# iDC-NEU/NeutronStarLite

Measured on AMD Instinct MI355X. Metric: aggregated_edges_per_sec, higher is better.
Workload: dtype f32; 1 GPU; reddit: RMAT V=232965 E=114232965 feat=602 GCN-layer aggregation fwd+bwd (BASELINE config #2); model=gcn, V=232965, E=114232965, feat=602, relabel=none, parallelism=graph-partitioned dp1

## Files before the change

include/nts_hip.h:

```cpp
#ifndef NTS_HIP_H
#define NTS_HIP_H

#include <stdint.h>

#ifdef __cplusplus
extern "C" {
#endif

typedef uint32_t nts_vid;

typedef struct nts_stream nts_stream;

nts_stream *nts_stream_create(void);
nts_stream *nts_stream_wrap(void *hip_stream);
void nts_stream_destroy(nts_stream *s);
void nts_stream_sync(nts_stream *s);
void *nts_stream_handle(nts_stream *s);
void nts_stream_wait_stream(nts_stream *waiter, nts_stream *waitee);

enum nts_ktag {
  NTS_KTAG_FWD = 0,
  NTS_KTAG_BWD = 1,
  NTS_KTAG_DESER = 2,
  NTS_KTAG_AGGMSG = 3,
// ... 70 lines not shown
    int *grid, unsigned long long *scratch_bytes);

enum nts_gather_sched {
  NTS_SCHED_ITEM = 0,
  NTS_SCHED_PHASE = 1,
  NTS_SCHED_XCD = 2
};

void nts_gather_schedule(nts_stream *s, int schedule, int window_floats);

void nts_gather_schedule_last(nts_stream *s, int *schedule, int *window_floats);

void nts_gather_plan(nts_vid feature_size, unsigned alignment_bytes,
    nts_vid rows, nts_vid batch_size, nts_vid edges, int schedule_req,
    int window_req, int *schedule, int *window_floats, int *lane_group,
    int *vector_width, int *grid, int *blocked);

void nts_gather_plan_bf16(nts_vid feature_size, unsigned alignment_bytes,
    nts_vid rows, nts_vid batch_size, nts_vid edges, int schedule_req,
    int window_req, int *schedule, int *window_floats, int *lane_group,
    int *vector_width, int *grid, int *blocked);

void nts_gather_staging(nts_stream *s, int mode);

void nts_gather_staging_last(nts_stream *s, int *staged, int *pitch_floats);

void nts_gather_stage_plan(nts_vid feature_size, unsigned elem_bytes,
    unsigned in_alignment_bytes, unsigned out_alignment_bytes, nts_vid rows,
    nts_vid batch_size, nts_vid edges, int schedule_req, int window_req,
    int stage_req, int *staged, int *pitch_floats, int *schedule,
    int *window_floats, int *lane_group, int *vector_width, int *store_width,
    int *grid, int *blocked);

void nts_items_cache_clear(nts_stream *s);

void nts_deserialize_to_gpu(nts_stream *s, float *gpu_buffer, const float *msg,
    nts_vid count, nts_vid feature_size, nts_vid partition_start,
    nts_vid partition_end, int sync);

void nts_aggregate_comm_result(nts_stream *s, float *master, const float *msg,
    nts_vid count, nts_vid feature_size, nts_vid partition_start,
    nts_vid partition_end, int sync);

void nts_gather_rows(nts_stream *s, const float *dense, float *packed,
    const nts_vid *index, nts_vid count, nts_vid row_start, nts_vid feature_size);
void nts_scatter_rows(nts_stream *s, float *dense, const float *packed,
    const nts_vid *index, nts_vid count, nts_vid row_start, nts_vid feature_size);
void nts_scatter_add_rows(nts_stream *s, float *dense, const float *packed,
    const nts_vid *index, nts_vid count, nts_vid row_start, nts_vid feature_size);

void nts_scatter_src_mirror_to_msg(nts_stream *s, float *message,
    const float *src_mirror_feature, const nts_vid *row_indices,
    const nts_vid *column_offset, const nts_vid *mirror_index,
    nts_vid batch_size, nts_vid feature_size);
void nts_gather_msg_to_src_mirror(nts_stream *s, float *src_mirror_feature,
    const float *message, const nts_vid *row_indices,
    const nts_vid *column_offset, const nts_vid *mirror_index,
    nts_vid batch_size, nts_vid feature_size);
void nts_scatter_dst_to_msg(nts_stream *s, float *message,
    const float *dst_feature, const nts_vid *row_indices,
    const nts_vid *column_offset, nts_vid batch_size, nts_vid feature_size);
void nts_gather_msg_to_dst(nts_stream *s, float *dst_feature,
    const float *message, const nts_vid *row_indices,
    const nts_vid *column_offset, nts_vid batch_size, nts_vid feature_size);

void nts_edge_softmax_forward(nts_stream *s, float *msg_output,
// ... 84 lines not shown
```

neutronstarlite_amd/csrc/nts_hip.hip:

```cpp
#include <hip/hip_runtime.h>

#include <cstdio>
#include <cstdlib>
#include <cstring>
#include <map>
#include <utility>
#include <vector>

#include "../../include/nts_hip.h"

#define NTS_CHECK(cmd)                                                        \
  do {                                                                        \
    hipError_t e_ = (cmd);                                                    \
    if (e_ != hipSuccess) {                                                   \
      fprintf(stderr, "nts_hip: %s failed: %s (%s:%d)\n", #cmd,               \
              hipGetErrorString(e_), __FILE__, __LINE__);                     \
      abort();          \
    }                                                                         \
  } while (0)

namespace {
constexpr int NTS_BLOCK = 256;

uint32_t env_u32(const char *name, uint32_t dflt) {
// ... 21 lines not shown
  uint4 *items = nullptr;
  uint32_t *counter = nullptr;
  uint64_t cap = 0;
  const uint32_t *key_off = nullptr;
  uint32_t key_batch = 0, key_edges = 0;
  bool valid = false;
};
}

struct nts_stream {
  hipStream_t stream = nullptr;
  bool owned = false;
  bool timing = false;
  struct Rec { hipEvent_t a, b; int tag; };
  std::vector<Rec> pending;
  std::vector<std::pair<hipEvent_t, hipEvent_t>> freeev;
  double acc_ns[NTS_KTAG_COUNT] = {};
  long long acc_n[NTS_KTAG_COUNT] = {};
  ItemsBuf items_scratch[2];
  int items_rr = 0;
  bool items_reuse = false;
  int sched_req = 0, window_req = 0;
  int sched_last = 0, window_last = 0;
  float *sums_ws = nullptr;
  uint64_t sums_cap = 0;
  unsigned long long *keys_ws = nullptr;
  uint64_t keys_cap = 0;
  float *stage_ws = nullptr;
  uint64_t stage_cap = 0;
  int stage_req = 0;
  bool staged_last = false;
  uint32_t stage_ld_last = 0;
  bool heads_general = false;
};

namespace {
struct Tic {
  nts_stream *s;
  int tag;
  hipEvent_t a = nullptr, b = nullptr;
  Tic(nts_stream *s_, int tag_) : s(s_), tag(tag_) {
    if (!s->timing) return;
    if (!s->freeev.empty()) {
      a = s->freeev.back().first;
      b = s->freeev.back().second;
      s->freeev.pop_back();
    } else {
      NTS_CHECK(hipEventCreate(&a));
      NTS_CHECK(hipEventCreate(&b));
    }
    NTS_CHECK(hipEventRecord(a, s->stream));
  }
  ~Tic() {
    if (!s->timing || !a) return;
    NTS_CHECK(hipEventRecord(b, s->stream));
    s->pending.push_back({a, b, tag});
  }
};

void drain_timing(nts_stream *s) {
  if (s->pending.empty()) return;
  NTS_CHECK(hipStreamSynchronize(s->stream));
  for (auto &r : s->pending) {
    float ms = 0.f;
    NTS_CHECK(hipEventElapsedTime(&ms, r.a, r.b));
    s->acc_ns[r.tag] += (double)ms * 1e6;
// ... 319 lines not shown
          for (int j = 0; j < nv; ++j) acc[j] = fmaf(w, to_f32(p[j]), acc[j]);
        }
      }
      if (nv > 0)
        store_acc<ELEM, OV>(out + (uint64_t)im.v * f + col, acc, nv,
                            im.shared);
    }
  }
}

template <int SV>
__global__ __launch_bounds__(NTS_BLOCK) void k_repitch(
    const float *__restrict__ src, float *__restrict__ dst, uint32_t rows,
    uint32_t f, uint32_t ld) {
  const WaveId w = wave_id();
  for (uint32_t r = w.wave; r < rows; r += w.n_waves) {
    const float *s = src + (uint64_t)r * f;
    float *d = dst + (uint64_t)r * ld;
    for (uint32_t c = w.lane * 4; c < f; c += 64 * 4) {
      fvec<4> v;
      if (c + 4 <= f) {
#pragma unroll
        for (int k = 0; k < 4 / SV; ++k) {
          const fvec<SV> x = *reinterpret_cast<const fvec<SV> *>(s + c + k * SV);
#pragma unroll
          for (int j = 0; j < SV; ++j) v[k * SV + j] = x[j];
        }
      } else {
#pragma unroll
        for (int j = 0; j < 4; ++j) v[j] = (c + j < f) ? s[c + j] : 0.f;
      }
      *reinterpret_cast<fvec<4> *>(d + c) = v;
    }
  }
}

template <int ELEM, int NE>
__device__ __forceinline__ void heads_edges_vec(float (&acc)[ELEM],
                                                const GatherSrc<float> &g,
                                                uint32_t e, uint32_t col,
                                                uint32_t K, uint32_t head) {
  const float *p[NE];
  float wv[NE];
#pragma unroll
  for (int k = 0; k < NE; ++k) {
    p[k] = g.in + (uint64_t)(g.nbr[e + k] - g.nbr_start) * g.ld + col;
    wv[k] = g.ew[(uint64_t)(e + k) * K + head];
  }
  fma_vec<ELEM, NE>(acc, p, wv);
}
template <int NSTR, int NE>
__device__ __forceinline__ void heads_edges_strided(
    float (&acc)[NSTR], const GatherSrc<float> &g, uint32_t e, uint32_t col,
    uint32_t G, uint32_t K, const uint32_t (&hd)[NSTR]) {
  const float *p[NE];
  const float *wrow[NE];
#pragma unroll
  for (int k = 0; k < NE; ++k) {
    p[k] = g.in + (uint64_t)(g.nbr[e + k] - g.nbr_start) * g.ld + col;
    wrow[k] = g.ew + (uint64_t)(e + k) * K;
  }
#pragma unroll
  for (int k = 0; k < NE; ++k)
#pragma unroll
    for (int j = 0; j < NSTR; ++j)
      if (col + j * G < g.f)
// ... 958 lines not shown
  NTS_CHECK(hipMemsetAsync(ib.counter, 0, sizeof(uint32_t), s->stream));
  {
    Tic t(s, NTS_KTAG_ITEMS);
    hipLaunchKernelGGL(k_build_items, dim3(grid_for(batch)), dim3(NTS_BLOCK), 0,
                       s->stream, offset, batch, NTS_SPLIT, ib.items,
                       ib.counter);
  }
  dbg_sync(s, "k_build_items");
  ib.key_off = offset;
  ib.key_batch = batch;
  ib.key_edges = edges;
  ib.valid = s->items_reuse;
  return ib;
}

uint32_t items_grid(uint32_t batch, uint32_t edges) {
  return grid_for(((uint64_t)batch + edges / NTS_SPLIT) * 64);
}

constexpr uint64_t NTS_BLOCK_MIN_BYTES = 256ull << 20;
constexpr uint32_t NTS_BLOCK_MIN_REUSE = 32;
constexpr int NTS_AUTO_SCHED = NTS_SCHED_PHASE;
constexpr uint32_t NTS_AUTO_WINDOW = 0;
constexpr int NTS_AUTO_SCHED_BF16 = NTS_SCHED_XCD;
constexpr uint32_t NTS_AUTO_WINDOW_BF16 = 302;
constexpr int NTS_AUTO_SCHED_STAGED = NTS_SCHED_PHASE;
constexpr uint32_t NTS_AUTO_WINDOW_STAGED = 128;

struct GatherEnv {
  bool forced = false;
  int sched = 0, window = 0;
  int stage = 0;
  uint32_t stage_pitch = 0;
  uint32_t split, max_blocks, gather_blocks;
};
const GatherEnv &gather_env() {
  static const GatherEnv env = [] {
    GatherEnv v;
    const char *e = getenv("NTS_GATHER_SCHED");
    if (e && *e && atoi(e) >= 0) {
      v.forced = true;
      v.sched = atoi(e);
      const char *w = getenv("NTS_GATHER_WINDOW");
      if (w && *w) v.window = atoi(w);
    }
    const char *st = getenv("NTS_GATHER_STAGE");
    if (st && *st) v.stage = atoi(st) > 0 ? 1 : atoi(st) < 0 ? -1 : 0;
    v.stage_pitch = env_u32("NTS_GATHER_STAGE_PITCH", 0);
    v.split = NTS_SPLIT;
    v.max_blocks = NTS_MAX_BLOCKS;
    v.gather_blocks = nts_gather_blocks();
    return v;
  }();
  return env;
}

struct GatherGeom { int elem, nstr; uint32_t G; };
GatherGeom gather_geometry(uint32_t f, uintptr_t alignment,
                           uint32_t elem_bytes, uint32_t also_divides = 0) {
  GatherGeom g;
  g.elem = 1;
  for (uint32_t bytes = 16; bytes > elem_bytes; bytes /= 2) {
    const uint32_t n = bytes / elem_bytes;
    if (f % n == 0 && alignment % bytes == 0 &&
        (!also_divides || also_divides % n == 0)) {
      g.elem = (int)n;
      break;
    }
  }
  g.nstr = (g.elem == 1) ? 4 : 1;
  const uint32_t unit = g.elem * g.nstr;
  const uint32_t need = (f + unit - 1) / unit;
  g.G = 64;
  while (g.G / 2 >= need && g.G > 16) g.G /= 2;
  return g;
}

struct GatherLaunch {
  int elem;
  uint32_t G, grid;
  bool blocked;
// ... 90 lines not shown
};
StagePlan plan_stage(uint32_t f, uint32_t elem_bytes, uintptr_t in_alignment,
                     uintptr_t out_alignment, uint32_t rows, uint32_t batch,
                     uint32_t edges, int sched_req, int window_req,
                     int stage_req, const GatherEnv &env) {
  const int req = stage_req ? stage_req : env.stage;
  const uint32_t unit =
      env.stage_pitch ? (env.stage_pitch + 3u) / 4u * 4u : NTS_STAGE_PITCH_UNIT;
  const uint64_t ld = ((uint64_t)f + unit - 1) / unit * unit;
  bool staged = elem_bytes == sizeof(float) && rows && req >= 0 &&
                ld <= 0xffffffffu &&
                (uint64_t)rows * ld * sizeof(float) <= NTS_STAGE_MAX_BYTES;
  if (staged && req == 0) {
    const GatherGeom native =
        gather_geometry(f, in_alignment | out_alignment, elem_bytes);
    const uint32_t slabf = native.G * native.elem * native.nstr;
    staged = ld != f && f > slabf &&
             (uint64_t)rows * f * elem_bytes > NTS_BLOCK_MIN_BYTES &&
             edges / NTS_STAGE_MIN_REUSE >= rows;
  }
  if (!staged) {
    const GatherLaunch L =
        plan_gather(f, in_alignment | out_alignment, elem_bytes, rows, batch,
                    edges, sched_req, window_req, env);
    return StagePlan{false, f, common_ov(L.elem, (int)elem_bytes), L};
  }
  GatherGeom geo{4, 1, 64};
  while (geo.G / 2 >= (f + 3) / 4 && geo.G > 16) geo.G /= 2;
  return StagePlan{true, (uint32_t)ld, stage_store_width(f, out_alignment),
                   plan_gather(geo, f, elem_bytes, rows, batch, edges,
                               sched_req, window_req, env, true)};
}

float *get_stage(nts_stream *s, uint64_t n) {
  if (s->stage_cap < n) {
    NTS_CHECK(hipStreamSynchronize(s->stream));
    if (s->stage_ws) NTS_CHECK(hipFree(s->stage_ws));
    s->stage_ws = nullptr;
    s->stage_cap = 0;
    NTS_CHECK(hipMalloc(&s->stage_ws, n * sizeof(float)));
    s->stage_cap = n;
  }
  return s->stage_ws;
}

template <typename T>
void launch_gather(nts_stream *s, const T *in, float *out, const float *ew,
                   const uint32_t *nbr, const uint32_t *offset,
                   uint32_t nbr_start, uint32_t batch, uint32_t edges,
                   uint32_t f, int with_weight, int tag, uint32_t rows) {
  if (!batch || !edges || !f) return;
  ItemsBuf &ib = get_items(s, offset, batch, edges);
  const StagePlan P = plan_stage(f, sizeof(T), (uintptr_t)in, (uintptr_t)out,
                                 rows, batch, edges, s->sched_req,
                                 s->window_req, s->stage_req, gather_env());
  const GatherLaunch &L = P.L;
  using Kernel = decltype(&k_gather_spmm<T, 1, false, false>);
#define NTS_K(E)                                                              \
  {{k_gather_spmm<T, E, false, false>, k_gather_spmm<T, E, false, true>},     \
   {k_gather_spmm<T, E, true, false>, k_gather_spmm<T, E, true, true>}}
  constexpr int WIDEST = 16 / (int)sizeof(T);
  static const Kernel kernels[4][2][2] = {NTS_K(1), NTS_K(2), NTS_K(4),
                                          NTS_K(WIDEST)};
#undef NTS_K
  s->sched_last = (int)L.pl.sched;
  s->window_last = (int)L.pl.wf;
  s->staged_last = P.staged;
  s->stage_ld_last = P.staged ? P.ld : 0;
  if constexpr (sizeof(T) == sizeof(float)) {
    if (P.staged) {
#define NTS_K(OV)                                                             \
  {{k_gather_spmm<float, 4, false, false, OV>,                                \
    k_gather_spmm<float, 4, false, true, OV>},                                \
   {k_gather_spmm<float, 4, true, false, OV>,                                 \
    k_gather_spmm<float, 4, true, true, OV>}}
      static const Kernel staged_kernels[3][2][2] = {NTS_K(1), NTS_K(2),
                                                     NTS_K(4)};
#undef NTS_K
      float *stage = get_stage(s, (uint64_t)rows * P.ld);
      const int sv = stage_store_width(f, (uintptr_t)in);
      Tic t(s, tag);
      hipLaunchKernelGGL(sv == 4   ? k_repitch<4>
                         : sv == 2 ? k_repitch<2>
                                   : k_repitch<1>,
                         dim3(grid_for((uint64_t)rows * 64)), dim3(NTS_BLOCK),
                         0, s->stream, in, stage, rows, f, P.ld);
      hipLaunchKernelGGL(staged_kernels[__builtin_ctz((unsigned)P.ov)]
                                       [with_weight != 0][L.blocked],
                         dim3(L.grid), dim3(NTS_BLOCK), 0, s->stream, ib.items,
                         ib.counter, nbr, ew, (const float *)stage, out,
                         nbr_start, f, P.ld, L.G, L.pl);
      dbg_sync(s, "k_gather_spmm (staged)");
      return;
    }
  }
  Tic t(s, tag);
  hipLaunchKernelGGL(kernels[__builtin_ctz((unsigned)L.elem)]
                            [with_weight != 0][L.blocked],
                     dim3(L.grid), dim3(NTS_BLOCK), 0, s->stream, ib.items,
                     ib.counter, nbr, ew, in, out, nbr_start, f, f, L.G, L.pl);
  dbg_sync(s, "k_gather_spmm");
}

void check_heads(const char *entry, uint32_t f, uint32_t heads) {
  if (heads == 0 || heads > f || f % heads != 0) {
    fprintf(stderr, "%s: heads %u does not divide feature_size %u\n", entry,
            heads, f);
    abort();
  }
}

GatherLaunch plan_gather_heads(uint32_t f, uint32_t heads, uintptr_t alignment,
                               uint32_t batch, uint32_t edges,
                               const GatherEnv &env) {
  const GatherGeom geo =
      gather_geometry(f, alignment, sizeof(float), f / heads);
  const uint32_t slabf = geo.G * geo.elem * geo.nstr;
  const uint32_t n_slabs = (f + slabf - 1) / slabf;
  const uint64_t bound_items = (uint64_t)batch + edges / env.split + 1;
  return GatherLaunch{
      geo.elem, geo.G,
      grid_for(bound_items * n_slabs * geo.G, env.max_blocks), false,
      GatherPlan{NTS_SCHED_ITEM, slabf, n_slabs, 1u}};
}

void launch_gather_heads(nts_stream *s, const char *entry, const float *in,
                         float *out, const float *ew, const uint32_t *nbr,
                         const uint32_t *offset, uint32_t nbr_start,
                         uint32_t batch, uint32_t edges, uint32_t f,
                         uint32_t heads, int tag, uint32_t rows) {
  check_heads(entry, f, heads);
  if (heads == 1) {
    launch_gather(s, in, out, ew, nbr, offset, nbr_start, batch, edges, f, 1,
                  tag, rows);
    return;
  }
  if (!batch || !edges) return;
  ItemsBuf &ib = get_items(s, offset, batch, edges);
  const GatherLaunch L = plan_gather_heads(
      f, heads, (uintptr_t)in | (uintptr_t)out, batch, edges, gather_env());
  s->sched_last = (int)L.pl.sched;
  s->window_last = (int)L.pl.wf;
  Tic t(s, tag);
  hipLaunchKernelGGL(L.elem == 4   ? k_gather_spmm_heads<4>
                     : L.elem == 2 ? k_gather_spmm_heads<2>
                                   : k_gather_spmm_heads<1>,
                     dim3(L.grid), dim3(NTS_BLOCK), 0, s->stream, ib.items,
                     ib.counter, nbr, ew, in, out, nbr_start, f, L.G,
                     L.pl.n_windows, heads, f / heads);
  dbg_sync(s, "k_gather_spmm_heads");
}

void check_reduce_op(const char *entry, int op) {
  if (op != NTS_REDUCE_MAX && op != NTS_REDUCE_MIN) {
    fprintf(stderr, "%s: op %d is neither NTS_REDUCE_MAX nor NTS_REDUCE_MIN\n",
            entry, op);
    abort();
  }
}

struct ReduceLaunch {
  GatherLaunch L;
  uint64_t key_elems;
};
ReduceLaunch plan_reduce(uint32_t f, uintptr_t alignment, uint32_t batch,
                         uint32_t edges, const GatherEnv &env) {
  ReduceLaunch r{};
  if (!batch || !edges || !f) return r;
  r.L = plan_gather(f, alignment, sizeof(float), batch, batch, edges,
                    NTS_SCHED_ITEM, -1, env);
  r.key_elems = edges > env.split ? (uint64_t)batch * f : 0;
  return r;
}

unsigned long long *get_keys(nts_stream *s, uint64_t n) {
  if (s->keys_cap < n) {
    NTS_CHECK(hipStreamSynchronize(s->stream));
    if (s->keys_ws) NTS_CHECK(hipFree(s->keys_ws));
    NTS_CHECK(hipMalloc(&s->keys_ws, n * sizeof(unsigned long long)));
    s->keys_cap = n;
  }
  return s->keys_ws;
}

void launch_reduce(nts_stream *s, int op, const float *in, float *out,
                   uint32_t *arg, const uint32_t *nbr, const uint32_t *offset,
                   uint32_t nbr_start, uint32_t batch, uint32_t edges,
                   uint32_t f) {
  check_reduce_op("nts_reduce_by_dst_from_src", op);
  if (!batch || !f) return;
  const ReduceLaunch R = plan_reduce(
      f, (uintptr_t)in | (uintptr_t)out | (uintptr_t)arg, batch, edges,
      gather_env());
  ItemsBuf *ib = edges ? &get_items(s, offset, batch, edges) : nullptr;
  unsigned long long *keys = R.key_elems ? get_keys(s, R.key_elems) : nullptr;
  const uint32_t row_grid = grid_for((uint64_t)batch * 64);
  s->sched_last = NTS_SCHED_ITEM;
  s->window_last = (int)R.L.pl.wf;
  Tic t(s, NTS_KTAG_FWD);
  hipLaunchKernelGGL((k_reduce_rows<false, false>), dim3(row_grid),
                     dim3(NTS_BLOCK), 0, s->stream, offset, batch, NTS_SPLIT,
                     out, arg, keys, f);
  if (ib) {
    using Kernel = decltype(&k_gather_reduce<1, false, false>);
#define NTS_K(E)                                                              \
  {{k_gather_reduce<E, false, false>, k_gather_reduce<E, false, true>},       \
   {k_gather_reduce<E, true, false>, k_gather_reduce<E, true, true>}}
    static const Kernel kernels[3][2][2] = {NTS_K(1), NTS_K(2), NTS_K(4)};
#undef NTS_K
    hipLaunchKernelGGL(
        kernels[__builtin_ctz((unsigned)R.L.elem)][op == NTS_REDUCE_MIN]
               [nbr == nullptr],
        dim3(R.L.grid), dim3(NTS_BLOCK), 0, s->stream, ib->items, ib->counter,
        nbr, in, out, arg, keys, nbr_start, f, R.L.G, R.L.pl.n_windows);
  }
  if (keys)
    hipLaunchKernelGGL((op == NTS_REDUCE_MIN ? k_reduce_rows<true, true>
                                             : k_reduce_rows<true, false>),
                       dim3(row_grid), dim3(NTS_BLOCK), 0, s->stream, offset,
                       batch, NTS_SPLIT, out, arg, keys, f);
  dbg_sync(s, "k_gather_reduce");
}
}

extern "C" {

nts_stream *nts_stream_create(void) {
  nts_stream *s = new nts_stream();
  NTS_CHECK(hipStreamCreateWithFlags(&s->stream, hipStreamNonBlocking));
  s->owned = true;
  return s;
// ... 268 lines not shown

void nts_gather_staging(nts_stream *s, int mode) {
  s->stage_req = mode > 0 ? 1 : mode < 0 ? -1 : 0;
}

void nts_gather_staging_last(nts_stream *s, int *staged, int *pitch_floats) {
  if (staged) *staged = s->staged_last ? 1 : 0;
  if (pitch_floats) *pitch_floats = (int)s->stage_ld_last;
}

void nts_gather_stage_plan(nts_vid feature_size, unsigned elem_bytes,
                           unsigned in_alignment_bytes,
                           unsigned out_alignment_bytes, nts_vid rows,
                           nts_vid batch_size, nts_vid edges, int schedule_req,
                           int window_req, int stage_req, int *staged,
                           int *pitch_floats, int *schedule,
                           int *window_floats, int *lane_group,
                           int *vector_width, int *store_width, int *grid,
                           int *blocked) {
  StagePlan P{};
  if (batch_size && edges && feature_size)
    P = plan_stage(feature_size, elem_bytes, in_alignment_bytes,
                   out_alignment_bytes, rows, batch_size, edges, schedule_req,
                   window_req, stage_req, gather_env());
  if (staged) *staged = P.staged ? 1 : 0;
  if (pitch_floats) *pitch_floats = (int)P.ld;
  if (schedule) *schedule = (int)P.L.pl.sched;
  if (window_floats) *window_floats = (int)P.L.pl.wf;
  if (lane_group) *lane_group = (int)P.L.G;
  if (vector_width) *vector_width = P.L.elem;
  if (store_width) *store_width = P.ov;
  if (grid) *grid = (int)P.L.grid;
  if (blocked) *blocked = P.L.blocked ? 1 : 0;
}

void nts_items_cache_clear(nts_stream *s) {
  NTS_CHECK(hipStreamSynchronize(s->stream));
  for (auto &slot : s->items_scratch) slot.valid = false;
}

void nts_items_reuse(nts_stream *s, int enable) {
  if (!enable) nts_items_cache_clear(s);
  s->items_reuse = enable != 0;
}

void nts_deserialize_to_gpu(nts_stream *s, float *gpu_buffer, const float *msg,
                            nts_vid count, nts_vid feature_size,
                            nts_vid partition_start, nts_vid partition_end,
                            int sync) {
  (void)partition_end;
  if (count) {
    Tic t(s, NTS_KTAG_DESER);
    hipLaunchKernelGGL(k_deserialize,
                       dim3(grid_for((uint64_t)count * feature_size)),
                       dim3(NTS_BLOCK), 0, s->stream, msg, count,
                       partition_start, gpu_buffer, feature_size);
  }
  if (sync) NTS_CHECK(hipStreamSynchronize(s->stream));
}

void nts_aggregate_comm_result(nts_stream *s, float *master, const float *msg,
                               nts_vid count, nts_vid feature_size,
                               nts_vid partition_start, nts_vid partition_end,
                               int sync) {
  (void)partition_end;
  if (count) {
// ... 471 lines not shown
```

neutronstarlite_amd/shim.py:

```python
import atexit
import ctypes
import os
import weakref

_DIR = os.path.dirname(os.path.abspath(__file__))
_SO = os.path.join(_DIR, "libnts_hip.so")

KTAG_FWD = 0
KTAG_BWD = 1
KTAG_DESER = 2
KTAG_AGGMSG = 3
KTAG_ITEMS = 4
KTAG_EDGE = 5

_c = ctypes
_vp = _c.c_void_p
_u32 = _c.c_uint32
_i32 = _c.c_int
_i64 = _c.c_long


class NtsHipMissing(RuntimeError):
    pass

# ... 19 lines not shown
    l.nts_stream_handle.restype = _vp
    l.nts_stream_handle.argtypes = [_vp]
    l.nts_stream_timing.argtypes = [_vp, _i32]
    l.nts_stream_timing_reset.argtypes = [_vp]
    l.nts_stream_kernel_ns.restype = _c.c_double
    l.nts_stream_kernel_ns.argtypes = [_vp, _i32]
    l.nts_stream_kernel_launches.restype = _c.c_longlong
    l.nts_stream_kernel_launches.argtypes = [_vp, _i32]
    l.nts_malloc_gpu.restype = _vp
    l.nts_malloc_gpu.argtypes = [_i64]
    l.nts_malloc_pinned.restype = _vp
    l.nts_malloc_pinned.argtypes = [_i64]
    l.nts_get_device_pointer.restype = _vp
    l.nts_get_device_pointer.argtypes = [_vp]
    l.nts_free_gpu.argtypes = [_vp]
    l.nts_free_host.argtypes = [_vp]
    l.nts_zero_buffer.argtypes = [_vp, _vp, _i64]
    l.nts_memcpy_h2d.argtypes = [_vp, _vp, _vp, _i64, _i32]
    l.nts_memcpy_d2h.argtypes = [_vp, _vp, _vp, _i64, _i32]
    l.nts_gather_by_dst_from_src.argtypes = [_vp] + [_vp] * 5 + [_u32] * 7 + [_i32]
    l.nts_gather_by_src_from_dst.argtypes = [_vp] + [_vp] * 5 + [_u32] * 7 + [_i32]
    l.nts_gather_by_dst_from_src_bf16.argtypes = (
        l.nts_gather_by_dst_from_src.argtypes)
    l.nts_gather_by_src_from_dst_bf16.argtypes = (
        l.nts_gather_by_src_from_dst.argtypes)
    l.nts_items_cache_clear.argtypes = [_vp]
    l.nts_gather_schedule.argtypes = [_vp, _i32, _i32]
    l.nts_gather_schedule_last.argtypes = [_vp, _vp, _vp]
    l.nts_gather_plan.argtypes = [_u32] * 5 + [_i32] * 2 + [_vp] * 6
    l.nts_gather_plan_bf16.argtypes = l.nts_gather_plan.argtypes
    l.nts_gather_staging.argtypes = [_vp, _i32]
    l.nts_gather_staging_last.argtypes = [_vp, _vp, _vp]
    l.nts_gather_stage_plan.argtypes = [_u32] * 7 + [_i32] * 3 + [_vp] * 9
    l.nts_deserialize_to_gpu.argtypes = [_vp, _vp, _vp, _u32, _u32, _u32, _u32, _i32]
    l.nts_aggregate_comm_result.argtypes = [_vp, _vp, _vp, _u32, _u32, _u32, _u32, _i32]
    l.nts_gather_rows.argtypes = [_vp, _vp, _vp, _vp, _u32, _u32, _u32]
    l.nts_scatter_rows.argtypes = [_vp, _vp, _vp, _vp, _u32, _u32, _u32]
    l.nts_scatter_add_rows.argtypes = [_vp, _vp, _vp, _vp, _u32, _u32, _u32]
    l.nts_scatter_src_mirror_to_msg.argtypes = [_vp] + [_vp] * 5 + [_u32] * 2
    l.nts_gather_msg_to_src_mirror.argtypes = [_vp] + [_vp] * 5 + [_u32] * 2
    l.nts_scatter_dst_to_msg.argtypes = [_vp] + [_vp] * 4 + [_u32] * 2
    l.nts_gather_msg_to_dst.argtypes = [_vp] + [_vp] * 4 + [_u32] * 2
    l.nts_scatter_grad_back_to_message.argtypes = [_vp] + [_vp] * 4 + [_u32] * 2
    l.nts_edge_dot.argtypes = [_vp] + [_vp] * 5 + [_u32] * 3
    l.nts_edge_softmax_forward.argtypes = [_vp] + [_vp] * 5 + [_u32] * 2
    l.nts_edge_softmax_backward.argtypes = [_vp] + [_vp] * 5 + [_u32] * 2
    l.nts_edge_softmax_forward_dual.argtypes = [_vp] + [_vp] * 6 + [_u32] * 2
    l.nts_edge_softmax_backward_fused.argtypes = (
        [_vp] + [_vp] * 6 + [_c.c_float] + [_vp] * 2 + [_u32] * 2)
    l.nts_gather_by_src_from_dst_dot.argtypes = (
        [_vp] + [_vp] * 5 + [_u32] * 4 + [_vp] * 3)
    l.nts_gather_by_src_from_dst_dot.restype = _i32
    l.nts_edge_attention_forward.argtypes = (
        [_vp] + [_vp] * 8 + [_c.c_float] + [_vp] + [_u32])
    l.nts_gather_by_dst_from_src_heads.argtypes = (
        [_vp] + [_vp] * 5 + [_u32] * 8)
    l.nts_gather_by_src_from_dst_heads.argtypes = (
        l.nts_gather_by_dst_from_src_heads.argtypes)
    l.nts_gather_plan_heads.argtypes = [_u32] * 5 + [_vp] * 3
    l.nts_edge_attention_forward_heads.argtypes = (
        [_vp] + [_vp] * 8 + [_c.c_float] + [_vp] + [_u32] * 3)
    l.nts_edge_dot_heads.argtypes = [_vp] + [_vp] * 5 + [_u32] * 5
    l.nts_weight_sum_heads.argtypes = [_vp] + [_vp] * 3 + [_u32] * 3
    l.nts_heads_dbg_general.argtypes = [_vp, _i32]
    l.nts_reduce_by_dst_from_src.argtypes = (
        [_vp, _i32] + [_vp] * 5 + [_u32] * 7)
# ... 17 lines not shown
             "blocked")
    out = [_i32(0) for _ in names]
    entry(f, alignment, rows, batch, edges, schedule, window,
          *[_c.byref(o) for o in out])
    plan = {n: o.value for n, o in zip(names, out)}
    plan["blocked"] = bool(plan["blocked"])
    return plan


def gather_plan(f, alignment, rows, batch, edges, schedule=0, window=0):
    return _plan(lib().nts_gather_plan, f, alignment, rows, batch, edges,
                 schedule, window)


def gather_plan_bf16(f, alignment, rows, batch, edges, schedule=0, window=0):
    return _plan(lib().nts_gather_plan_bf16, f, alignment, rows, batch, edges,
                 schedule, window)


def gather_stage_plan(f, in_alignment, out_alignment, rows, batch, edges,
                      schedule=0, window=0, stage=0, elem_bytes=4):
    names = ("staged", "pitch", "schedule", "window", "lane_group",
             "vector_width", "store_width", "grid", "blocked")
    out = [_i32(0) for _ in names]
    lib().nts_gather_stage_plan(f, elem_bytes, in_alignment, out_alignment,
                                rows, batch, edges, schedule, window, stage,
                                *[_c.byref(o) for o in out])
    plan = {n: o.value for n, o in zip(names, out)}
    plan["staged"] = bool(plan["staged"])
    plan["blocked"] = bool(plan["blocked"])
    return plan


def check_heads(f, heads):
    if not (isinstance(heads, int) and isinstance(f, int)
            and 1 <= heads <= f and f % heads == 0):
        raise ValueError(
            f"heads={heads!r} must be a positive divisor of the width {f!r}")


def gather_plan_heads(f, heads, alignment, batch, edges):
    check_heads(f, heads)
    names = ("lane_group", "vector_width", "grid")
    out = [_i32(0) for _ in names]
    lib().nts_gather_plan_heads(f, heads, alignment, batch, edges,
                                *[_c.byref(o) for o in out])
    return {n: o.value for n, o in zip(names, out)}


REDUCE_OPS = {"max": 0, "min": 1}
NO_EDGE = 0xFFFFFFFF


def reduce_op(op):
    if not isinstance(op, str) or op not in REDUCE_OPS:
        raise ValueError(f"op={op!r} must be 'max' or 'min'")
    return REDUCE_OPS[op]


def reduce_plan(f, alignment, batch, edges, op="max"):
    reduce_op(op)
    names = ("lane_group", "vector_width", "grid")
    out = [_i32(0) for _ in names]
    scratch = _c.c_ulonglong(0)
    lib().nts_reduce_plan(f, alignment, batch, edges,
                          *[_c.byref(o) for o in out], _c.byref(scratch))
# ... 181 lines not shown

    def sample_reservoir(self, column_offset, row_indices, dst_list, n_dst,
                         fanout, seed, out_src, out_cnt):
        self._lib.nts_sample_reservoir(self.h, _vp(column_offset),
                                       _vp(row_indices), _vp(dst_list),
                                       n_dst, fanout, seed, _vp(out_src),
                                       _vp(out_cnt))

    def sample_reservoir_dbg_fallback(self, column_offset, row_indices,
                                      dst_list, n_dst, fanout, seed,
                                      out_src, out_cnt):
        self._lib.nts_sample_reservoir_dbg_fallback(
            self.h, _vp(column_offset), _vp(row_indices), _vp(dst_list),
            n_dst, fanout, seed, _vp(out_src), _vp(out_cnt))

    def gather_schedule(self, schedule=0, window_floats=0):
        self._lib.nts_gather_schedule(self.h, schedule, window_floats)

    def gather_schedule_last(self):
        sched, window = _i32(0), _i32(0)
        self._lib.nts_gather_schedule_last(self.h, _c.byref(sched),
                                           _c.byref(window))
        return sched.value, window.value

    def gather_staging(self, mode=0):
        self._lib.nts_gather_staging(self.h, mode)

    def gather_staging_last(self):
        staged, pitch = _i32(0), _i32(0)
        self._lib.nts_gather_staging_last(self.h, _c.byref(staged),
                                          _c.byref(pitch))
        return bool(staged.value), pitch.value

    def items_cache_clear(self):
        self._lib.nts_items_cache_clear(self.h)

    def items_reuse(self, enable):
        self._lib.nts_items_reuse(self.h, 1 if enable else 0)

    def weight_sum(self, out, weights, offset, batch):
        self._lib.nts_weight_sum(self.h, _vp(out), _vp(weights), _vp(offset),
                                 batch)

    def edge_attention_forward(self, softmax_out, softmax_out_perm, perm_pos,
                               m_sum_out, s_src_mirror, s_dst, row_indices,
                               mirror_index, slope, column_offset, batch):
        self._lib.nts_edge_attention_forward(
            self.h, _vp(softmax_out), _vp(softmax_out_perm), _vp(perm_pos),
            _vp(m_sum_out), _vp(s_src_mirror), _vp(s_dst), _vp(row_indices),
            _vp(mirror_index), slope, _vp(column_offset), batch)

    def gather_by_dst_from_src_heads(self, x_ptr, y_ptr, w_ptr,
                                     row_indices_ptr, column_offset_ptr,
                                     src_s, src_e, dst_s, dst_e, edges, batch,
                                     f, heads):
        check_heads(f, heads)
        self._lib.nts_gather_by_dst_from_src_heads(
            self.h, _vp(x_ptr), _vp(y_ptr), _vp(w_ptr), _vp(row_indices_ptr),
            _vp(column_offset_ptr), src_s, src_e, dst_s, dst_e, edges, batch,
            f, heads)

    def gather_by_src_from_dst_heads(self, g_ptr, y_ptr, w_ptr,
                                     row_offset_ptr, column_indices_ptr,
                                     src_s, src_e, dst_s, dst_e, edges, batch,
                                     f, heads):
        check_heads(f, heads)
# ... 51 lines not shown
```

Baseline: 5.116 billion edges/s.

## Add striped staged gather kernel mapping windows to XCD-aligned stripes

Adds a new staged SpMM gather kernel that splits each feature window into narrower column stripes and assigns (item, stripe) tasks to waves. The block index modulo 8 chooses the stripe class, so each block class keeps revisiting the same column slice, and each wave runs a fixed number of tasks in sequence. Edges are spread across subgroups of lanes and combined with cross-lane shuffles. By default this path is taken whenever the auto plan picks the staged phase schedule, which raises the risk of regressions from the different work partitioning and extra reductions.

```diff
diff --git a/cpp/stripe_plan_check.cpp b/cpp/stripe_plan_check.cpp
--- /dev/null
+++ b/cpp/stripe_plan_check.cpp
@@ -0,0 +1,58 @@
+#include <cstdio>
+#include <set>
+#include <utility>
+#include <vector>
+
+#include "../include/nts_hip.h"
+
+static int fail(const char *what, unsigned n, unsigned f, unsigned sf) {
+  fprintf(stderr, "stripe_plan_check FAIL: %s (n_items %u f %u stripe %u)\n",
+          what, n, f, sf);
+  return 1;
+}
+
+int main() {
+  const unsigned items[] = {1, 7, 8, 9, 1000, 1001};
+  const unsigned widths[] = {32, 130, 602, 608};
+  const unsigned stripes[] = {16, 32, 64, 128};
+  const int runs[] = {0, 3, 17};
+  const unsigned window = 128;
+  long checked = 0;
+  for (unsigned n : items)
+    for (unsigned f : widths)
+      for (unsigned sf : stripes)
+        for (int run : runs) {
+          int grid = 0, stripe = 0, per_wave = 0, staged = 0;
+          nts_gather_stripe_plan(f, 4, 16, 16, n, n, n, NTS_SCHED_PHASE,
+                                 (int)window, 1, (int)sf, run, &staged,
+                                 nullptr, nullptr, nullptr, nullptr, nullptr,
+                                 nullptr, &grid, nullptr, &stripe, nullptr,
+                                 nullptr, nullptr, &per_wave);
+          if (!staged || stripe != (int)sf || grid < 8 || grid % 8 ||
+              per_wave < (run ? run : 1))
+            return fail("plan", n, f, sf);
+          const unsigned long long slots =
+              (unsigned long long)grid * 4 * per_wave;
+          std::vector<nts_vid> it(slots + 16), c0(slots + 16), c1(slots + 16);
+          const long long live = nts_gather_stripe_task(
+              f, 4, 16, 16, n, n, n, NTS_SCHED_PHASE, (int)window, 1, (int)sf,
+              run, n, 0, slots + 16, it.data(), c0.data(), c1.data());
+          std::set<std::pair<nts_vid, nts_vid>> seen;
+          for (unsigned long long k = 0; k < slots + 16; ++k) {
+            if (c0[k] >= c1[k]) continue;
+            if (k >= slots) return fail("task past the grid", n, f, sf);
+            const nts_vid bound = c0[k] + sf < f ? c0[k] + sf : f;
+            if (it[k] >= n || c0[k] >= f || c0[k] % sf || c1[k] != bound)
+              return fail("task outside the rows", n, f, sf);
+            if (!seen.insert({it[k], c0[k]}).second)
+              return fail("task twice", n, f, sf);
+          }
+          const unsigned long long want =
+              (unsigned long long)n * ((f + sf - 1) / sf);
+          if ((unsigned long long)live != want || seen.size() != want)
+            return fail("tasks missing", n, f, sf);
+          ++checked;
+        }
+  printf("stripe_plan_check ok (%ld launches)\n", checked);
+  return 0;
+}
diff --git a/include/nts_hip.h b/include/nts_hip.h
--- a/include/nts_hip.h
+++ b/include/nts_hip.h
@@ -126,6 +126,29 @@
     int *window_floats, int *lane_group, int *vector_width, int *store_width,
     int *grid, int *blocked);
 
+void nts_gather_stripes(nts_stream *s, int stripe_floats);
+
+void nts_gather_stripes_run(nts_stream *s, int tasks_per_wave);
+
+void nts_gather_stripes_last(nts_stream *s, int *stripe_floats,
+    int *tasks_per_wave);
+
+void nts_gather_stripe_plan(nts_vid feature_size, unsigned elem_bytes,
+    unsigned in_alignment_bytes, unsigned out_alignment_bytes, nts_vid rows,
+    nts_vid batch_size, nts_vid edges, int schedule_req, int window_req,
+    int stage_req, int stripe_req, int run_req, int *staged,
+    int *pitch_floats, int *schedule, int *window_floats, int *lane_group,
+    int *vector_width, int *store_width, int *grid, int *blocked,
+    int *stripe_floats, int *stripe_lanes, int *subgroups, int *stripes,
+    int *tasks_per_wave);
+
+long long nts_gather_stripe_task(nts_vid feature_size, unsigned elem_bytes,
+    unsigned in_alignment_bytes, unsigned out_alignment_bytes, nts_vid rows,
+    nts_vid batch_size, nts_vid edges, int schedule_req, int window_req,
+    int stage_req, int stripe_req, int run_req, nts_vid n_items,
+    unsigned long long first_slot, unsigned long long count, nts_vid *item,
+    nts_vid *first_column, nts_vid *column_bound);
+
 void nts_items_cache_clear(nts_stream *s);
 
 void nts_deserialize_to_gpu(nts_stream *s, float *gpu_buffer, const float *msg,
diff --git a/neutronstarlite_amd/csrc/nts_hip.hip b/neutronstarlite_amd/csrc/nts_hip.hip
--- a/neutronstarlite_amd/csrc/nts_hip.hip
+++ b/neutronstarlite_amd/csrc/nts_hip.hip
@@ -77,6 +77,9 @@
   bool staged_last = false;
   uint32_t stage_ld_last = 0;
   bool heads_general = false;
+  int stripe_req = 0;
+  int stripe_run_req = 0;
+  uint32_t stripe_last = 0, stripe_run_last = 0;
 };
 
 namespace {
@@ -462,6 +465,130 @@
       }
       *reinterpret_cast<fvec<4> *>(d + c) = v;
     }
+  }
+}
+
+struct StripePlan {
+  uint32_t wf;
+  uint32_t sf;
+  uint32_t S;
+  uint32_t R;
+  uint32_t n_windows;
+  uint32_t n_full;
+  uint32_t last_live;
+};
+
+__host__ __device__ inline void stripe_divmod(uint64_t a, uint32_t b,
+                                              uint64_t &q, uint32_t &r) {
+  if (a <= 0xffffffffu) {
+    q = (uint32_t)a / b;
+    r = (uint32_t)a % b;
+  } else {
+    q = a / b;
+    r = (uint32_t)(a % b);
+  }
+}
+
+__host__ __device__ inline Task stripe_task(uint32_t grid, uint32_t n_items,
+                                            uint32_t f, const StripePlan &sp,
+                                            uint32_t block, uint32_t wave,
+                                            uint32_t run) {
+  const Task none{0u, 0u, 0u};
+  if (block >= grid || run >= sp.R) return none;
+  const uint32_t cls = block & 7u, cpw = 8u / sp.S;
+  const uint32_t stripe = cls % sp.S, sub = cls / sp.S;
+  const uint64_t t =
+      ((uint64_t)(block >> 3) * (NTS_BLOCK / 64) + wave) * sp.R + run;
+  const uint32_t ni = n_items > sub ? (n_items - sub + cpw - 1) / cpw : 0u;
+  const uint64_t own = (uint64_t)sp.n_full * ni;
+  uint32_t it, win, st;
+  if (t < own) {
+    uint64_t w;
+    uint32_t slot;
+    stripe_divmod(t, ni, w, slot);
+    win = (uint32_t)w;
+    it = sub + cpw * slot;
+    st = stripe;
+  } else {
+    if (!sp.last_live) return none;
+    const uint64_t u = cls + 8u * (t - own);
+    if (u >= (uint64_t)n_items * sp.last_live) return none;
+    uint64_t q;
+    stripe_divmod(u, sp.last_live, q, st);
+    it = (uint32_t)q;
+    win = sp.n_windows - 1;
+  }
+  const uint32_t fbase = win * sp.wf + st * sp.sf;
+  const uint32_t fend = fbase + sp.sf;
+  return Task{it, fbase, fend < f ? fend : f};
+}
+
+template <int ELEM, bool WITH_W, bool FULL>
+__device__ __forceinline__ void stripe_edges(float (&acc)[ELEM],
+                                             const GatherSrc<float> &g,
+                                             uint32_t eb, uint32_t e_end,
+                                             uint32_t sub, uint32_t P,
+                                             uint32_t col) {
+  uint32_t idx[4];
+  float wv[4];
+  bool live[4];
+#pragma unroll
+  for (int k = 0; k < 4; ++k) {
+    uint32_t e = eb + k * P + sub;
+    live[k] = FULL || e < e_end;
+    if (!FULL) e = min(e, e_end - 1);
+    idx[k] = g.nbr[e];
+    wv[k] = WITH_W ? g.ew[e] : 1.0f;
+  }
+  float x[4][ELEM];
+#pragma unroll
+  for (int k = 0; k < 4; ++k)
+    load_lane<ELEM>(g.in + (uint64_t)(idx[k] - g.nbr_start) * g.ld + col,
+                    x[k]);
+#pragma unroll
+  for (int k = 0; k < 4; ++k)
+    if (live[k]) {
+#pragma unroll
+      for (int j = 0; j < ELEM; ++j) acc[j] = fmaf(wv[k], x[k][j], acc[j]);
+    }
+}
+
+template <int ELEM, bool WITH_W, int OV, int GS>
+__global__ __launch_bounds__(NTS_BLOCK) void k_gather_spmm_stripe(
+    const uint4 *__restrict__ items, const uint32_t *__restrict__ n_items_p,
+    const uint32_t *__restrict__ nbr, const float *__restrict__ ew,
+    const float *__restrict__ in, float *__restrict__ out, uint32_t nbr_start,
+    uint32_t f, uint32_t ld, StripePlan sp) {
+  static_assert(GS >= 4 && GS <= 64 && (GS & (GS - 1)) == 0, "lanes a stripe");
+  constexpr uint32_t P = 64 / GS;
+  const uint32_t n_items = *n_items_p;
+  const uint32_t lane = threadIdx.x & 63u;
+  const uint32_t sub = lane / GS, glane = lane % GS;
+  const uint32_t wave = threadIdx.x >> 6;
+  const GatherSrc<float> g{nbr, ew, in, nbr_start, f, ld};
+  for (uint32_t run = 0; run < sp.R; ++run) {
+    const Task tk =
+        stripe_task(gridDim.x, n_items, f, sp, blockIdx.x, wave, run);
+    if (tk.fbase >= tk.fend) continue;
+    const Item im = load_item(items, tk.it);
+    const uint32_t col = tk.fbase + glane * ELEM;
+    const int nv = (col + ELEM <= tk.fend)
+                       ? ELEM : (col < tk.fend ? (int)(tk.fend - col) : 0);
+    float acc[ELEM] = {};
+    if (nv > 0) {
+      const uint32_t e_end = im.e0 + im.cnt;
+      uint32_t eb = im.e0;
+      for (; eb + 4 * P <= e_end; eb += 4 * P)
+        stripe_edges<ELEM, WITH_W, true>(acc, g, eb, e_end, sub, P, col);
+      if (eb < e_end)
+        stripe_edges<ELEM, WITH_W, false>(acc, g, eb, e_end, sub, P, col);
+    }
+#pragma unroll
+    for (int w = 32; w >= GS; w >>= 1)
+#pragma unroll
+      for (int j = 0; j < ELEM; ++j) acc[j] += __shfl_xor(acc[j], w, 64);
+    if (sub == 0 && nv > 0)
+      store_acc<ELEM, OV>(out + (uint64_t)im.v * f + col, acc, nv, im.shared);
   }
 }
 
@@ -1486,6 +1613,8 @@
   int sched = 0, window = 0;
   int stage = 0;
   uint32_t stage_pitch = 0;
+  int stripe = 0;
+  uint32_t stripe_run = 0;
   uint32_t split, max_blocks, gather_blocks;
 };
 const GatherEnv &gather_env() {
@@ -1501,6 +1630,9 @@
     const char *st = getenv("NTS_GATHER_STAGE");
     if (st && *st) v.stage = atoi(st) > 0 ? 1 : atoi(st) < 0 ? -1 : 0;
     v.stage_pitch = env_u32("NTS_GATHER_STAGE_PITCH", 0);
+    const char *sp = getenv("NTS_GATHER_STRIPE");
+    if (sp && *sp) v.stripe = atoi(sp) < 0 ? -1 : atoi(sp);
+    v.stripe_run = env_u32("NTS_GATHER_STRIPE_RUN", 0);
     v.split = NTS_SPLIT;
     v.max_blocks = NTS_MAX_BLOCKS;
     v.gather_blocks = nts_gather_blocks();
@@ -1657,6 +1789,79 @@
                                sched_req, window_req, env, true)};
 }
 
+constexpr uint32_t NTS_AUTO_STRIPE_STAGED = 64;
+constexpr uint32_t NTS_AUTO_STRIPE_RUN = 16;
+
+struct StripeLaunch {
+  bool on;
+  uint32_t Gs, P, grid;
+  StripePlan sp;
+};
+StripeLaunch plan_stripe(const StagePlan &P, uint32_t f, uint32_t elem_bytes,
+                         uint32_t batch, uint32_t edges, int sched_req,
+                         int window_req, int stage_req, int stripe_req,
+                         int run_req, const GatherEnv &env) {
+  StripeLaunch off{};
+  const int req = stripe_req ? stripe_req : env.stripe;
+  if (req < 0 || !P.staged || elem_bytes != sizeof(float)) return off;
+  int rs = 0;
+  uint32_t rw = 0;
+  bool asked = false;
+  if (sched_req || window_req) {
+    asked = true;
+    rs = sched_req;
+    rw = window_req > 0 ? (uint32_t)window_req : 0;
+  } else if (env.forced) {
+    asked = true;
+    rs = env.sched;
+    rw = env.window > 0 ? (uint32_t)env.window : 0;
+  }
+  const bool phase = P.L.blocked && P.L.pl.sched == NTS_SCHED_PHASE;
+  uint32_t sf, wf = P.L.pl.wf;
+  if (req == 0) {
+    if (asked || stage_req || env.stage || !phase) return off;
+    sf = NTS_AUTO_STRIPE_STAGED;
+  } else {
+    if (!phase && !(asked && rs == NTS_SCHED_PHASE)) return off;
+    if (!P.L.blocked && rw) wf = (rw + 3u) / 4u * 4u;
+    sf = (uint32_t)req;
+  }
+  if (!sf || sf % 4u || wf % sf) return off;
+  const uint32_t S = wf / sf, Gs = sf / 4u;
+  if (S != 1 && S != 2 && S != 4 && S != 8) return off;
+  if (Gs < 4 || Gs > 64 || (Gs & (Gs - 1))) return off;
+  const uint32_t cap8 = env.gather_blocks & ~7u;
+  if (cap8 < 8) return off;
+
+  StripePlan sp{};
+  sp.wf = wf;
+  sp.sf = sf;
+  sp.S = S;
+  sp.n_windows = (f + wf - 1) / wf;
+  const uint32_t last_w = f - (sp.n_windows - 1) * wf;
+  const uint32_t last_live = (last_w + sf - 1) / sf;
+  sp.n_full = last_live == S ? sp.n_windows : sp.n_windows - 1;
+  sp.last_live = last_live == S ? 0u : last_live;
+  const uint64_t bound_items = (uint64_t)batch + edges / env.split + 1;
+  const uint32_t cpw = 8u / S;
+  const uint64_t tasks = (uint64_t)sp.n_full * ((bound_items + cpw - 1) / cpw) +
+                         (bound_items * sp.last_live + 7u) / 8u;
+  const uint64_t waves_cap = (uint64_t)(cap8 / 8u) * (NTS_BLOCK / 64);
+  uint64_t R = (tasks + waves_cap - 1) / waves_cap;
+  const uint32_t want = run_req > 0       ? (uint32_t)run_req
+                        : env.stripe_run ? env.stripe_run
+                        : req == 0       ? NTS_AUTO_STRIPE_RUN
+                                         : 0u;
+  if (R < want) R = want;
+  if (R < 1) R = 1;
+  if (R > 0xffffffffu) return off;
+  sp.R = (uint32_t)R;
+  const uint64_t waves = (tasks + R - 1) / R;
+  uint64_t blocks = (waves + NTS_BLOCK / 64 - 1) / (NTS_BLOCK / 64);
+  if (blocks < 1) blocks = 1;
+  return StripeLaunch{true, Gs, 64u / Gs, (uint32_t)(blocks * 8u), sp};
+}
+
 float *get_stage(nts_stream *s, uint64_t n) {
   if (s->stage_cap < n) {
     NTS_CHECK(hipStreamSynchronize(s->stream));
@@ -1664,6 +1869,11 @@
     s->stage_ws = nullptr;
     s->stage_cap = 0;
     NTS_CHECK(hipMalloc(&s->stage_ws, n * sizeof(float)));
+    if ((uintptr_t)s->stage_ws % 128 != 0) {
+      fprintf(stderr, "nts_hip: staging buffer %p is not 128-byte aligned\n",
+              (void *)s->stage_ws);
+      abort();
+    }
     s->stage_cap = n;
   }
   return s->stage_ws;
@@ -1692,6 +1902,7 @@
   s->window_last = (int)L.pl.wf;
   s->staged_last = P.staged;
   s->stage_ld_last = P.staged ? P.ld : 0;
+  s->stripe_last = s->stripe_run_last = 0;
   if constexpr (sizeof(T) == sizeof(float)) {
     if (P.staged) {
 #define NTS_K(OV)                                                             \
@@ -1710,6 +1921,32 @@
                                    : k_repitch<1>,
                          dim3(grid_for((uint64_t)rows * 64)), dim3(NTS_BLOCK),
                          0, s->stream, in, stage, rows, f, P.ld);
+      const StripeLaunch SL = plan_stripe(
+          P, f, sizeof(T), batch, edges, s->sched_req, s->window_req,
+          s->stage_req, s->stripe_req, s->stripe_run_req, gather_env());
+      if (SL.on) {
+        using SKernel = decltype(&k_gather_spmm_stripe<4, false, 1, 4>);
+#define NTS_K(OV, GS)                                                         \
+  {k_gather_spmm_stripe<4, false, OV, GS>, k_gather_spmm_stripe<4, true, OV, GS>}
+#define NTS_KG(OV)                                                            \
+  {NTS_K(OV, 4), NTS_K(OV, 8), NTS_K(OV, 16), NTS_K(OV, 32), NTS_K(OV, 64)}
+        static const SKernel stripe_kernels[3][5][2] = {NTS_KG(1), NTS_KG(2),
+                                                        NTS_KG(4)};
+#undef NTS_KG
+#undef NTS_K
+        s->sched_last = NTS_SCHED_PHASE;
+        s->window_last = (int)SL.sp.wf;
+        s->stripe_last = SL.sp.sf;
+        s->stripe_run_last = SL.sp.R;
+        hipLaunchKernelGGL(stripe_kernels[__builtin_ctz((unsigned)P.ov)]
+                                         [__builtin_ctz(SL.Gs) - 2]
+                                         [with_weight != 0],
+                           dim3(SL.grid), dim3(NTS_BLOCK), 0, s->stream,
+                           ib.items, ib.counter, nbr, ew, (const float *)stage,
+                           out, nbr_start, f, P.ld, SL.sp);
+        dbg_sync(s, "k_gather_spmm_stripe");
+        return;
+      }
       hipLaunchKernelGGL(staged_kernels[__builtin_ctz((unsigned)P.ov)]
                                        [with_weight != 0][L.blocked],
                          dim3(L.grid), dim3(NTS_BLOCK), 0, s->stream, ib.items,
@@ -1766,6 +2003,7 @@
       f, heads, (uintptr_t)in | (uintptr_t)out, batch, edges, gather_env());
   s->sched_last = (int)L.pl.sched;
   s->window_last = (int)L.pl.wf;
+  s->stripe_last = s->stripe_run_last = 0;
   Tic t(s, tag);
   hipLaunchKernelGGL(L.elem == 4   ? k_gather_spmm_heads<4>
                      : L.elem == 2 ? k_gather_spmm_heads<2>
@@ -1822,6 +2060,7 @@
   const uint32_t row_grid = grid_for((uint64_t)batch * 64);
   s->sched_last = NTS_SCHED_ITEM;
   s->window_last = (int)R.L.pl.wf;
+  s->stripe_last = s->stripe_run_last = 0;
   Tic t(s, NTS_KTAG_FWD);
   hipLaunchKernelGGL((k_reduce_rows<false, false>), dim3(row_grid),
                      dim3(NTS_BLOCK), 0, s->stream, offset, batch, NTS_SPLIT,
@@ -2156,6 +2395,102 @@
   if (store_width) *store_width = P.ov;
   if (grid) *grid = (int)P.L.grid;
   if (blocked) *blocked = P.L.blocked ? 1 : 0;
+}
+
+void nts_gather_stripes(nts_stream *s, int stripe_floats) {
+  s->stripe_req = stripe_floats < 0 ? -1 : stripe_floats;
+}
+
+void nts_gather_stripes_run(nts_stream *s, int tasks_per_wave) {
+  s->stripe_run_req = tasks_per_wave > 0 ? tasks_per_wave : 0;
+}
+
+void nts_gather_stripes_last(nts_stream *s, int *stripe_floats,
+                             int *tasks_per_wave) {
+  if (stripe_floats) *stripe_floats = (int)s->stripe_last;
+  if (tasks_per_wave) *tasks_per_wave = (int)s->stripe_run_last;
+}
+
+static StripeLaunch stripe_plan_of(nts_vid feature_size, unsigned elem_bytes,
+                                   unsigned in_alignment_bytes,
+                                   unsigned out_alignment_bytes, nts_vid rows,
+                                   nts_vid batch_size, nts_vid edges,
+                                   int schedule_req, int window_req,
+                                   int stage_req, int stripe_req, int run_req,
+                                   StagePlan &P) {
+  P = StagePlan{};
+  if (!batch_size || !edges || !feature_size)
+    return StripeLaunch{};
+  P = plan_stage(feature_size, elem_bytes, in_alignment_bytes,
+                 out_alignment_bytes, rows, batch_size, edges, schedule_req,
+                 window_req, stage_req, gather_env());
+  return plan_stripe(P, feature_size, elem_bytes, batch_size, edges,
+                     schedule_req, window_req, stage_req, stripe_req, run_req,
+                     gather_env());
+}
+
+void nts_gather_stripe_plan(nts_vid feature_size, unsigned elem_bytes,
+                            unsigned in_alignment_bytes,
+                            unsigned out_alignment_bytes, nts_vid rows,
+                            nts_vid batch_size, nts_vid edges, int schedule_req,
+                            int window_req, int stage_req, int stripe_req,
+                            int run_req, int *staged, int *pitch_floats,
+                            int *schedule, int *window_floats, int *lane_group,
+                            int *vector_width, int *store_width, int *grid,
+                            int *blocked, int *stripe_floats,
+                            int *stripe_lanes, int *subgroups, int *stripes,
+                            int *tasks_per_wave) {
+  StagePlan P;
+  const StripeLaunch SL = stripe_plan_of(
+      feature_size, elem_bytes, in_alignment_bytes, out_alignment_bytes, rows,
+      batch_size, edges, schedule_req, window_req, stage_req, stripe_req,
+      run_req, P);
+  if (staged) *staged = P.staged ? 1 : 0;
+  if (pitch_floats) *pitch_floats = (int)P.ld;
+  if (schedule) *schedule = SL.on ? (int)NTS_SCHED_PHASE : (int)P.L.pl.sched;
+  if (window_floats) *window_floats = (int)(SL.on ? SL.sp.wf : P.L.pl.wf);
+  if (lane_group) *lane_group = (int)(SL.on ? SL.Gs : P.L.G);
+  if (vector_width) *vector_width = P.L.elem;
+  if (store_width) *store_width = P.ov;
+  if (grid) *grid = (int)(SL.on ? SL.grid : P.L.grid);
+  if (blocked) *blocked = (SL.on || P.L.blocked) ? 1 : 0;
+  if (stripe_floats) *stripe_floats = (int)SL.sp.sf;
+  if (stripe_lanes) *stripe_lanes = (int)SL.Gs;
+  if (subgroups) *subgroups = (int)SL.P;
+  if (stripes) *stripes = (int)SL.sp.S;
+  if (tasks_per_wave) *tasks_per_wave = (int)SL.sp.R;
+}
+
+long long nts_gather_stripe_task(
+    nts_vid feature_size, unsigned elem_bytes, unsigned in_alignment_bytes,
+    unsigned out_alignment_bytes, nts_vid rows, nts_vid batch_size,
+    nts_vid edges, int schedule_req, int window_req, int stage_req,
+    int stripe_req, int run_req, nts_vid n_items, unsigned long long first_slot,
+    unsigned long long count, nts_vid *item, nts_vid *first_column,
+    nts_vid *column_bound) {
+  StagePlan P;
+  const StripeLaunch SL = stripe_plan_of(
+      feature_size, elem_bytes, in_alignment_bytes, out_alignment_bytes, rows,
+      batch_size, edges, schedule_req, window_req, stage_req, stripe_req,
+      run_req, P);
+  long long live = 0;
+  constexpr uint32_t WAVES = NTS_BLOCK / 64;
+  for (unsigned long long k = 0; k < count; ++k) {
+    Task tk{0u, 0u, 0u};
+    if (SL.on) {
+      const unsigned long long slot = first_slot + k;
+      const unsigned long long w = slot / SL.sp.R;
+      if (w / WAVES < SL.grid)
+        tk = stripe_task(SL.grid, n_items, feature_size, SL.sp,
+                         (uint32_t)(w / WAVES), (uint32_t)(w % WAVES),
+                         (uint32_t)(slot % SL.sp.R));
+    }
+    if (item) item[k] = tk.it;
+    if (first_column) first_column[k] = tk.fbase;
+    if (column_bound) column_bound[k] = tk.fend;
+    live += tk.fbase < tk.fend;
+  }
+  return live;
 }
 
 void nts_items_cache_clear(nts_stream *s) {
diff --git a/neutronstarlite_amd/shim.py b/neutronstarlite_amd/shim.py
--- a/neutronstarlite_amd/shim.py
+++ b/neutronstarlite_amd/shim.py
@@ -75,6 +75,13 @@
     l.nts_gather_staging.argtypes = [_vp, _i32]
     l.nts_gather_staging_last.argtypes = [_vp, _vp, _vp]
     l.nts_gather_stage_plan.argtypes = [_u32] * 7 + [_i32] * 3 + [_vp] * 9
+    l.nts_gather_stripes.argtypes = [_vp, _i32]
+    l.nts_gather_stripes_run.argtypes = [_vp, _i32]
+    l.nts_gather_stripes_last.argtypes = [_vp, _vp, _vp]
+    l.nts_gather_stripe_plan.argtypes = [_u32] * 7 + [_i32] * 5 + [_vp] * 14
+    l.nts_gather_stripe_task.argtypes = (
+        [_u32] * 7 + [_i32] * 5 + [_u32] + [_c.c_ulonglong] * 2 + [_vp] * 3)
+    l.nts_gather_stripe_task.restype = _c.c_longlong
     l.nts_deserialize_to_gpu.argtypes = [_vp, _vp, _vp, _u32, _u32, _u32, _u32, _i32]
     l.nts_aggregate_comm_result.argtypes = [_vp, _vp, _vp, _u32, _u32, _u32, _u32, _i32]
     l.nts_gather_rows.argtypes = [_vp, _vp, _vp, _vp, _u32, _u32, _u32]
@@ -158,6 +165,34 @@
     return plan
 
 
+def gather_stripe_plan(f, in_alignment, out_alignment, rows, batch, edges,
+                       schedule=0, window=0, stage=0, stripe=0, run=0,
+                       elem_bytes=4):
+    names = ("staged", "pitch", "schedule", "window", "lane_group",
+             "vector_width", "store_width", "grid", "blocked", "stripe",
+             "stripe_lanes", "subgroups", "stripes", "tasks_per_wave")
+    out = [_i32(0) for _ in names]
+    lib().nts_gather_stripe_plan(f, elem_bytes, in_alignment, out_alignment,
+                                 rows, batch, edges, schedule, window, stage,
+                                 stripe, run, *[_c.byref(o) for o in out])
+    plan = {n: o.value for n, o in zip(names, out)}
+    plan["staged"] = bool(plan["staged"])
+    plan["blocked"] = bool(plan["blocked"])
+    return plan
+
+
+def gather_stripe_tasks(f, in_alignment, out_alignment, rows, batch, edges,
+                        n_items, first_slot, count, schedule=0, window=0,
+                        stage=0, stripe=0, run=0, elem_bytes=4):
+    import numpy as np
+    arrs = [np.zeros(count, dtype=np.uint32) for _ in range(3)]
+    lib().nts_gather_stripe_task(f, elem_bytes, in_alignment, out_alignment,
+                                 rows, batch, edges, schedule, window, stage,
+                                 stripe, run, n_items, first_slot, count,
+                                 *[a.ctypes.data for a in arrs])
+    return tuple(arrs)
+
+
 def check_heads(f, heads):
     if not (isinstance(heads, int) and isinstance(f, int)
             and 1 <= heads <= f and f % heads == 0):
@@ -405,6 +440,15 @@
                                           _c.byref(pitch))
         return bool(staged.value), pitch.value
 
+    def gather_stripes(self, stripe_floats=0, tasks_per_wave=0):
+        self._lib.nts_gather_stripes(self.h, stripe_floats)
+        self._lib.nts_gather_stripes_run(self.h, tasks_per_wave)
+
+    def gather_stripes_last(self):
+        sf, run = _i32(0), _i32(0)
+        self._lib.nts_gather_stripes_last(self.h, _c.byref(sf), _c.byref(run))
+        return sf.value, run.value
+
     def items_cache_clear(self):
         self._lib.nts_items_cache_clear(self.h)
 
```

New measurement: 6.289 billion edges/s (median of 6 runs). 22.9% higher.
